# TheCacophonyProject/audio-analysis

Measured on AMD Instinct MI355X. Metric: audio-seconds classified/sec/GPU on 60 s mono; max|delta logit| vs CPU ref, higher is better.
Workload: dtype bf16x3; 1 GPU; config2: 64 windows/step (39 of clip A + 25 of clip B, 60 s 48 kHz mono), htk log-mel n_fft 4096 hop 640 160 mel + model1 CNN; model=model1, global_batch=64, seq_len=144000, parallelism=dp1, pipeline=2 batches in flight on 2 streams, clip_pairs=4 resident clip pairs in rotation, one per step

## Files before the change

audio-analysis_amd/csrc/aa_frontend.hip:

```cpp
#include "aa_common.h"
#include "aa_wavefft.h"

#include <algorithm>
#include <cmath>
#include <cstring>
#include <vector>

namespace aa {

constexpr int kStatSplit = 16;
constexpr int kFpb = 6;

struct FePlan {
    aa_fe_config cfg;
    int T = 0;
    int kmin = 0;
    int kmax = 0;
    int nfblk = 0;
    int nnz = 0;
    float* d_win = nullptr;
    float2* d_tw = nullptr;
    float2* d_tw2 = nullptr;
    int4* d_rows = nullptr;
    float* d_vals = nullptr;
    char* d_cimg = nullptr;
    int cimg_bytes = 0;
    StageTimer timer;
};

enum { FE_STAGE_STATS = 0, FE_STAGE_STFT = 1, FE_STAGE_DB = 2, FE_N_STAGES = 3 };

__global__ __launch_bounds__(256) void fe_stats(const float* __restrict__ pcm,
                                                const aa_window* __restrict__ wins,
                                                int win_len, float4* __restrict__ stats) {
    const int w = blockIdx.y;
    const aa_window d = wins[w];
    const int chunk = (win_len + kStatSplit - 1) / kStatSplit;
    const int i0 = blockIdx.x * chunk;
    const int i1 = min(win_len, i0 + chunk);
    float mn = INFINITY, mx = -INFINITY;
    int bad = 0;
    const int v0 = max(i0, d.pad_left);
    const int v1 = min(i1, d.pad_left + d.n_valid);
    if (i0 < i1 && !(v0 == i0 && v1 >= i1)) { mn = 0.f; mx = 0.f; }
    if (v0 < v1) {
        const float* p = pcm + d.src + (v0 - d.pad_left);
        const int n = v1 - v0;
        const int head = min(n, (int)((16 - ((uintptr_t)p & 15)) & 15) / 4);
        for (int i = threadIdx.x; i < head; i += blockDim.x) {
            float x = p[i];
            bad |= !isfinite(x);
            mn = fminf(mn, x);
            mx = fmaxf(mx, x);
        }
        const int nb = (n - head) / 4;
        const float4* q = reinterpret_cast<const float4*>(p + head);
        constexpr int U = 4;
        for (int i = threadIdx.x; i < nb; i += U * blockDim.x) {
            float4 x[U];
#pragma unroll
            for (int u = 0; u < U; ++u) x[u] = q[min(i + u * (int)blockDim.x, nb - 1)];
#pragma unroll
            for (int u = 0; u < U; ++u) {
                bad |= !isfinite(x[u].x) | !isfinite(x[u].y) | !isfinite(x[u].z) | !isfinite(x[u].w);
                mn = fminf(fminf(mn, x[u].x), fminf(x[u].y, fminf(x[u].z, x[u].w)));
                mx = fmaxf(fmaxf(mx, x[u].x), fmaxf(x[u].y, fmaxf(x[u].z, x[u].w)));
            }
        }
        for (int i = head + nb * 4 + threadIdx.x; i < n; i += blockDim.x) {
            float x = p[i];
            bad |= !isfinite(x);
            mn = fminf(mn, x);
            mx = fmaxf(mx, x);
        }
    }
    __shared__ float smn[4], smx[4];
    __shared__ int sbad[4];
    mn = wave_min(mn);
    mx = wave_max(mx);
    bad = wave_or(bad);
    const int wv = threadIdx.x >> 6;
    if ((threadIdx.x & 63) == 0) { smn[wv] = mn; smx[wv] = mx; sbad[wv] = bad; }
    __syncthreads();
    if (threadIdx.x == 0) {
        for (int k = 1; k < (int)(blockDim.x >> 6); ++k) {
            mn = fminf(mn, smn[k]);
            mx = fmaxf(mx, smx[k]);
            bad |= sbad[k];
        }
        stats[w * kStatSplit + blockIdx.x] = make_float4(mn, mx, (float)bad, 0.f);
    }
}

__device__ __forceinline__ int pidx(int i) { return i + (i >> 3); }

template <int NC, int R, int NT, int NS>
struct Pass {
    static constexpr int NB = NC / R;
    static constexpr int PER = (NB + NT - 1) / NT;
    float2 t[PER][R - 1];
    __device__ __forceinline__ void load(const float2* __restrict__ tw) {
#pragma unroll
        for (int b = 0; b < PER; ++b) {
            const int j = threadIdx.x + b * NT;
            const int k = j % NS;
#pragma unroll
            for (int r = 1; r < R; ++r)
                t[b][r - 1] = tw[(r * k * (NC / (NS * R))) & (NC - 1)];
        }
    }
    __device__ __forceinline__ void run(const float2* __restrict__ src, float2* __restrict__ dst) const {
#pragma unroll
        for (int b = 0; b < PER; ++b) {
            const int j = threadIdx.x + b * NT;
            if (NB % NT == 0 || j < NB) {
                float2 v[R];
#pragma unroll
                for (int r = 0; r < R; ++r) v[r] = src[pidx(j + r * NB)];
                if constexpr (NS > 1) {
#pragma unroll
                    for (int r = 1; r < R; ++r) v[r] = cmul(v[r], t[b][r - 1]);
                }
                if constexpr (R == 8) dft8(v);
                if constexpr (R == 4) dft4(v[0], v[1], v[2], v[3]);
                if constexpr (R == 2) dft2(v[0], v[1]);
                const int k = j % NS;
                const int o = (j / NS) * NS * R + k;
#pragma unroll
                for (int r = 0; r < R; ++r) dst[pidx(o + r * NS)] = v[r];
            }
        }
    }
};

__device__ __forceinline__ float normalize_sample(float x, float lo, float scale, float inv) {
    const float a = __fsub_rn(x, lo);
    const float q0 = __fmul_rn(a, inv);
    const float r = fmaf(-q0, scale, a);
    float y = fmaf(r, inv, q0);
    y = __fadd_rn(y, 0.000001f);
    y = __fsub_rn(y, 0.5f);
    return __fmul_rn(y, 2.0f);
}

enum { PM_GENERAL = 0, PM_ABS = 1, PM_SQUARE = 2 };
template <int PM>
__device__ __forceinline__ float pow_mag(float re, float im, float power) {
    const float m2 = fmaf(re, re, im * im);
    if constexpr (PM == PM_SQUARE) return m2;
    const float mag = __builtin_amdgcn_sqrtf(m2);
    if constexpr (PM == PM_ABS) return mag;
    else return powf(mag, power);
}

template <int NFFT, int PM>
__global__ __launch_bounds__(NFFT / 16) void fe_stft_mel(
    const float* __restrict__ pcm, const aa_window* __restrict__ wins, const float4* __restrict__ stats,
    const float* __restrict__ hann, const float2* __restrict__ tw, const float2* __restrict__ tw2,
    const int4* __restrict__ rows, const float* __restrict__ vals, int nnz, int win_len, int hop, int T,
    int n_mels, int kmin, int kmax, int normalize, float power, int nfblk, int n_items,
    float* __restrict__ melS, float* __restrict__ blkmax) {
    constexpr int NC = NFFT / 2;
    constexpr int NT = NC / 8;
    constexpr int R4 = NC / 512;
    static_assert(NC >= 1024 && NC <= 4096, "NFFT 2048..8192");
    constexpr int KREG = 4;
    extern __shared__ float lds[];
    float* seg = lds;
    const int seg_cap = ((kFpb - 1) * hop + NFFT + 3) & ~3;
    float2* bufA = reinterpret_cast<float2*>(lds + seg_cap);
    constexpr int NCP = NC + NC / 8;
    float2* bufB = bufA + NCP;
    float* melT = reinterpret_cast<float*>(bufB + NCP);
    int4* srows = reinterpret_cast<int4*>(melT + ((n_mels * kFpb + 3) & ~3));
    float* svals = reinterpret_cast<float*>(srows + n_mels);

    const int tid = threadIdx.x;
    float hw[8][2];
#pragma unroll
    for (int r = 0; r < 8; ++r) {
        const int n = tid + r * (NC / 8);
        const float2 h = reinterpret_cast<const float2*>(hann)[n];
        hw[r][0] = h.x;
        hw[r][1] = h.y;
    }
    Pass<NC, 8, NT, 8> p2;
    Pass<NC, 8, NT, 64> p3;
    Pass<NC, R4, NT, 512> p4;
    p2.load(tw);
    p3.load(tw);
    p4.load(tw);
    float2 w2r[KREG];
#pragma unroll
    for (int i = 0; i < KREG; ++i) {
        w2r[i] = tw2[min(kmin + tid + i * NT, kmax)];
    }
    for (int i = tid; i < n_mels; i += NT) srows[i] = rows[i];
    for (int i = tid; i < nnz; i += NT) svals[i] = vals[i];

    __syncthreads();
    for (int item = blockIdx.x; item < n_items; item += gridDim.x) {
    const int w = item / nfblk;
    const int fb = item - w * nfblk;
    const int f0 = fb * kFpb;
    const int nf = min(kFpb, T - f0);
    const int seg_len = (nf - 1) * hop + NFFT;
    const aa_window d = wins[w];
    float lo = INFINITY, hi = -INFINITY;
#pragma unroll
    for (int s = 0; s < kStatSplit; ++s) {
        float4 st = stats[w * kStatSplit + s];
        lo = fminf(lo, st.x);
        hi = fmaxf(hi, st.y);
    }
    const float scale = __fsub_rn(hi, lo);
    const float inv = __fdiv_rn(1.f, scale);

    const int base = f0 * hop - NFFT / 2;
    constexpr int SEGU = 8;
    const long long safe = d.n_valid > 0 ? d.src : 0;
    for (int q0 = 0; q0 < seg_len; q0 += SEGU * NT) {
        float raw[SEGU];
        bool ok[SEGU];
#pragma unroll
        for (int u = 0; u < SEGU; ++u) {
            const int q = q0 + u * NT + tid;
            const int i = base + q;
            const int rel = i - d.pad_left;
            ok[u] = q < seg_len && i >= 0 && i < win_len && rel >= 0 && rel < d.n_valid;
            raw[u] = pcm[ok[u] ? d.src + rel : safe];
        }
#pragma unroll
        for (int u = 0; u < SEGU; ++u) {
            const int q = q0 + u * NT + tid;
            const int i = base + q;
            if (q < seg_len) {
                float v = 0.f;
                if (i >= 0 && i < win_len) {
                    v = ok[u] ? raw[u] : 0.f;
                    if (normalize) v = normalize_sample(v, lo, scale, inv);
                }
                seg[q] = v;
            }
        }
    }
    __syncthreads();

    float bmax = 0.f;
    for (int f = 0; f < nf; ++f) {
        {
            const float* x = seg + f * hop;
            float2 v[8];
#pragma unroll
            for (int r = 0; r < 8; ++r) {
                const int n = tid + r * NT;
                v[r] = make_float2(x[2 * n] * hw[r][0], x[2 * n + 1] * hw[r][1]);
            }
            dft8(v);
#pragma unroll
            for (int r = 0; r < 8; ++r) bufA[pidx(tid * 8 + r)] = v[r];
        }
        __syncthreads();
        p2.run(bufA, bufB);
        __syncthreads();
        p3.run(bufB, bufA);
        __syncthreads();
        p4.run(bufA, bufB);
        __syncthreads();
        const float2* Z = bufB;
        float* Pf = reinterpret_cast<float*>(bufA);
        for (int i = 0; kmin + tid + i * NT <= kmax; ++i) {
            const int k = kmin + tid + i * NT;
            float re, im;
            if (k == 0 || k == NC) {
                const float2 z0 = Z[0];
                re = (k == 0) ? z0.x + z0.y : z0.x - z0.y;
                im = 0.f;
            } else {
                const float2 a = Z[pidx(k)];
                const float2 b = Z[pidx(NC - k)];
                const float2 E = make_float2(0.5f * (a.x + b.x), 0.5f * (a.y - b.y));
                const float2 O = make_float2(0.5f * (a.y + b.y), -0.5f * (a.x - b.x));
                float2 wk;
                if (i < KREG) {
                    wk = w2r[0];
#pragma unroll
                    for (int q = 1; q < KREG; ++q) if (i == q) wk = w2r[q];
                } else {
                    wk = tw2[k];
                }
                const float2 X = cadd(E, cmul(wk, O));
                re = X.x;
                im = X.y;
            }
            Pf[k - kmin] = pow_mag<PM>(re, im, power);
        }
        __syncthreads();
        for (int m = tid; m < n_mels; m += NT) {
            const int4 rw = srows[m];
            const float* wv = svals + rw.z;
            const float* pv = Pf + (rw.x - kmin);
            float s = 0.f;
            for (int i0 = 0; i0 < rw.y; i0 += 16) {
                float a[16], b[16];
#pragma unroll
                for (int i = 0; i < 16; ++i) {
                    const int ii = min(i0 + i, rw.y - 1);
                    a[i] = (i0 + i < rw.y) ? wv[ii] : 0.f;
                    b[i] = pv[ii];
                }
#pragma unroll
                for (int i = 0; i < 16; ++i) s = fmaf(a[i], b[i], s);
            }
            melT[m * kFpb + f] = s;
            bmax = fmaxf(bmax, s);
        }
        __syncthreads();
    }
    const float inv_nm = 1.0f / (float)n_mels;
    for (int idx = tid; idx < nf * n_mels; idx += NT) {
        const int f = (int)(((float)idx + 0.5f) * inv_nm), m = idx - f * n_mels;
        melS[((size_t)w * T + f0 + f) * n_mels + m] = melT[m * kFpb + f];
    }
    __shared__ float red[NT / 64];
    bmax = wave_max(bmax);
    if ((tid & 63) == 0) red[tid >> 6] = bmax;
    __syncthreads();
    if (tid == 0) {
        for (int k = 1; k < NT / 64; ++k) bmax = fmaxf(bmax, red[k]);
        blkmax[w * nfblk + fb] = bmax;
    }
    }
}

__host__ __device__ constexpr int fe_mel_slots(int n_mels) { return (n_mels + 63) / 64 * 64; }

#ifndef AA_FE_WPB
#define AA_FE_WPB 8
#endif
#ifndef AA_FE_MEL_G
#define AA_FE_MEL_G 2
#endif
#ifndef AA_FE_MEL_P
#define AA_FE_MEL_P 1
#endif
constexpr int kWpb = AA_FE_WPB;

constexpr int kFeStampPh = 8;
__device__ unsigned long long* fe_stamps = nullptr;
#define FE_STAMP(k)                                                              \
    if constexpr ((DIAG & 128) != 0) {                                           \
        const unsigned long long tn = __builtin_amdgcn_s_memtime();              \
        st_acc[k] += tn - st_prev;                                               \
        st_prev = tn;                                                            \
    }
template <int PM, int DIAG = 0>
__global__ __launch_bounds__(64 * kWpb) __attribute__((amdgpu_waves_per_eu(kWpb / 2, kWpb / 2))) void fe_stft_mel_4096(
    const float* __restrict__ pcm, const aa_window* __restrict__ wins, const float4* __restrict__ stats,
    const float2* __restrict__ tw, const float2* __restrict__ tw4096, const char* __restrict__ cimg,
    int cimg_bytes, int win_len, int hop, int T, int n_mels, int kmin, int kmax, int normalize, float power,
    int n_frames, float* __restrict__ melF, float* __restrict__ pmax) {
    constexpr int NC = 2048;
    extern __shared__ float lds[];
    const int tid = threadIdx.x;
    const int wave = __builtin_amdgcn_readfirstlane(tid >> 6), lane = tid & 63;
    char* cl = reinterpret_cast<char*>(lds);
    const int4* srows = reinterpret_cast<const int4*>(cl);
    const float* svals = reinterpret_cast<const float*>(srows + fe_mel_slots(n_mels));
    float2* wb = reinterpret_cast<float2*>(cl + cimg_bytes) + wave * kHalf;

    for (int g = wave; g < cimg_bytes / 1024; g += kWpb)
        __builtin_amdgcn_global_load_lds((const __attribute__((address_space(1))) void*)(cimg + g * 1024 + lane * 16),
                                         (__attribute__((address_space(3))) void*)(cl + g * 1024), 16, 0, 0);
    const int k1 = lane >> 1, h = lane & 1;
    float2 t1 = tw[lane];
    float2 t8 = tw[(8 * lane) & (NC - 1)];
    const float2 wk1 = tw4096[k1];
    const float2 te = tw4096[2 * lane], to = tw4096[2 * lane + 1];
    const float2 hwe = make_float2(te.x, -te.y), hwo = make_float2(to.x, -to.y);
    __syncthreads();
    unsigned long long st_acc[kFeStampPh] = {}, st_prev = 0;
    auto load_frame = [&](int fl, float2 (&yy)[32]) {
        const int wl = fl / T;
        const aa_window dl = wins[wl];
        const int i0l = (fl - wl * T) * hop - 2048;
        int l2l = 2 * lane;
        __asm__ volatile("" : "+v"(l2l));
        const __amdgpu_buffer_rsrc_t rs =
            __builtin_amdgcn_make_buffer_rsrc((void*)(pcm + dl.src), 0, dl.n_valid * 4, 0x00020000);
        const int offe = i0l - dl.pad_left + l2l;
        const int v0 = i0l - dl.pad_left;
        if (v0 >= 0 && v0 + 4096 <= dl.n_valid) {
#pragma unroll
            for (int r = 0; r < 32; ++r) {
                const uint2 v = __builtin_bit_cast(uint2, __builtin_amdgcn_raw_buffer_load_b64(rs, (offe + 128 * r) * 4, 0, 0));
                yy[r] = make_float2(__uint_as_float(v.x), __uint_as_float(v.y));
            }
        } else {
            int offo = offe + 1;
            __asm__ volatile("" : "+v"(offo));
#pragma unroll
            for (int r = 0; r < 32; ++r) yy[r] = make_float2(load_view(rs, offe + 128 * r), load_view(rs, offo + 128 * r));
        }
    };

    const int nbx = gridDim.x >> 3;
    const int xcd = blockIdx.x & 7;
    const int f_end = (int)((long long)(xcd + 1) * n_frames / 8);
    const int G = nbx * kWpb;
    const int f_first = (int)((long long)xcd * n_frames / 8) + wave * nbx + (blockIdx.x >> 3);
    for (int fi = f_first; fi < f_end; fi += G) {
        const int w = fi / T;
        const int t = fi - w * T;
        if constexpr ((DIAG & 128) != 0) st_prev = __builtin_amdgcn_s_memtime();
        float apow = 1.f, beta = 0.f;
        if (normalize) {
            float lo = INFINITY, hi = -INFINITY;
#pragma unroll
            for (int s = 0; s < kStatSplit; ++s) {
                const float4 st = stats[w * kStatSplit + s];
                lo = fminf(lo, st.x);
                hi = fmaxf(hi, st.y);
            }
            const float scale = __fsub_rn(hi, lo);
            const float a = __fdiv_rn(2.f, scale);
            apow = PM == PM_SQUARE ? a * a : PM == PM_ABS ? a : powf(a, power);
            beta = fmaf(scale, 0.000001f - 0.5f, -lo);
        }
        const int i0 = t * hop - 2048;
        int l2 = 2 * lane;
        __asm__ volatile("" : "+v"(l2));
        float2 wk = wk1;
        __asm__ volatile("" : "+v"(wk.x), "+v"(wk.y));
        float2 u[32];
        {
            float2 y[32];
            if constexpr ((DIAG & 1) != 0) {
#pragma unroll
                for (int r = 0; r < 32; ++r) y[r] = make_float2((float)(lane + r), (float)(t - r));
            } else {
                load_frame(fi, y);
            }
            if (normalize && (i0 < 0 || i0 + 4096 > win_len)) {
#pragma unroll
                for (int r = 0; r < 32; ++r) {
                    const int i = i0 + l2 + 128 * r;
                    y[r].x = (i >= 0 && i < win_len) ? y[r].x + beta : 0.f;
                    y[r].y = (i + 1 >= 0 && i + 1 < win_len) ? y[r].y + beta : 0.f;
                }
            }
            float2 he = hwe, ho = hwo;
            float hs = lane >= 32 ? -0.5f : 0.5f;
            __asm__ volatile("" : "+v"(he.x), "+v"(he.y), "+v"(ho.x), "+v"(ho.y), "+v"(hs));
#pragma unroll
            for (int r = 0; r < 32; ++r) {
                const float cr = kW32[r][0], sr = -kW32[r][1];
                const float ce = fmaf(he.x, cr, -he.y * sr), co = fmaf(ho.x, cr, -ho.y * sr);
                const float a = (r & 1) ? hs : 0.5f;
                y[r].x *= fmaf(-a, ce, a);
                y[r].y *= fmaf(-a, co, a);
            }
            FE_STAMP(0)
            if constexpr ((DIAG & 4) != 0) {
#pragma unroll
                for (int j = 0; j < 32; ++j) u[j] = y[j];
            } else {
                const unsigned up = lane >= 32 ? 0x80000000u : 0u;
                auto flip = [up](float2 v) {
                    return make_float2(__uint_as_float(__float_as_uint(v.x) ^ up),
                                       __uint_as_float(__float_as_uint(v.y) ^ up));
                };
                dft32(y);
                FE_STAMP(1)
                __asm__ volatile("" : "+v"(t1.x), "+v"(t1.y), "+v"(t8.x), "+v"(t8.y));
                float2 p1[8], p8[4];
                p1[0] = make_float2(1.f, 0.f);
                p1[1] = t1;
#pragma unroll
                for (int i = 2; i < 8; ++i) p1[i] = cmul(p1[i - 1], t1);
                {
                    const float2 q1 = t8, q2 = cmul(t8, t8), q3 = cmul(q2, t8);
                    const bool hi = lane >= 32;
                    p8[0] = hi ? q2 : make_float2(1.f, 0.f);
                    p8[1] = hi ? q3 : q1;
                    p8[2] = hi ? make_float2(1.f, 0.f) : q2;
                    p8[3] = hi ? q1 : q3;
                }
#pragma unroll
                for (int k = 0; k < 32; ++k) {
                    const float2 tk = (k & 7) == 0 ? p8[k >> 3] : cmul(p8[k >> 3], p1[k & 7]);
                    y[dperm(k)] = cmul(y[dperm(k)], tk);
                }
                FE_STAMP(2)
#pragma unroll
                for (int pass = 0; pass < 2; ++pass) {
#pragma unroll
                    for (int k = 0; k < 16; ++k) wb[k * kRow + lane] = y[dperm(16 * pass + k)];
                    wave_sync();
                    const float2* src = wb + (k1 & 15) * kRow + h + 32 * (((k1 >> 4) ^ pass) & 1);
#pragma unroll
                    for (int i = 0; i < 16; ++i) u[16 * pass + i] = src[2 * i];
                    wave_sync();
                }
                FE_STAMP(3)
                dft32(u);
#pragma unroll
                for (int k = 1; k < 32; k += 2) u[dperm(k)] = flip(u[dperm(k)]);
                FE_STAMP(4)
                const float sg = h ? -1.f : 1.f;
#pragma unroll
                for (int j = 0; j < 32; ++j) {
                    const float2 e = u[dperm(j)];
                    const float2 wj = wconst64(j);
                    const float2 g = h ? cmul(wj, e) : e;
                    const float2 rv = make_float2(swap_pair(g.x), swap_pair(g.y));
                    u[dperm(j)] = make_float2(fmaf(sg, g.x, rv.x), fmaf(sg, g.y, rv.y));
                }
                FE_STAMP(5)
            }
        }
        if (h && !(DIAG & 8)) {
#pragma unroll
            for (int j = 0; j < 32; ++j) wb[k1 + 32 * j] = u[dperm(j)];
        }
        wave_sync();
        float* Pt = reinterpret_cast<float*>(wb) + (2 * kHalf - 1);
        if (!(DIAG & 8)) {
            const float2* mb = wb + (32 - k1) - 512 * h;
            float* pk = Pt - k1 - 512 * h - 32 * 15;
            const float r2 = 0.70710678118654752440f;
            const float2 wkh = h ? make_float2(r2 * (wk.x + wk.y), r2 * (wk.y - wk.x)) : wk;
            float pw[16];
            float2 zm[16];
#pragma unroll
            for (int i = 0; i < 8; ++i) zm[i] = mb[32 * (31 - i)];
#pragma unroll
            for (int i = 0; i < 16; ++i) {
                if (i % 8 == 0 && i + 8 < 16) {
#pragma unroll
                    for (int k = i + 8; k < i + 16; ++k) zm[k] = mb[32 * (31 - k)];
                }
                const float2 hiv = u[dperm(16 + i)];
                const float2 oth = make_float2(swap_pair(hiv.x), swap_pair(hiv.y));
                const float2 a = h ? oth : u[dperm(i)];
                const float2 zb = zm[i];
                const float2 b = (i == 0 && k1 == 0 && !h) ? a : zb;
                const float2 E = make_float2(0.5f * (a.x + b.x), 0.5f * (a.y - b.y));
                const float2 O = make_float2(0.5f * (a.y + b.y), -0.5f * (a.x - b.x));
                float2 wj = cmul(wkh, wconst128(i));
                __asm__ volatile("" : "+v"(wj.x), "+v"(wj.y));
                const float2 X = cadd(E, cmul(wj, O));
                pw[i] = pow_mag<PM>(X.x, X.y, power);
            }
            if (!(DIAG & 16)) {
#pragma unroll
                for (int i = 0; i < 16; ++i) pk[32 * (15 - i)] = pw[i];
            }
        }
        wave_sync();
        FE_STAMP(6)
        float fmx = 0.f;
        float* orow = melF + (size_t)fi * n_mels;
        const int nslot = fe_mel_slots(n_mels);
#if AA_FE_MEL_G > 0
        int si0 = lane;
        __asm__ volatile("" : "+v"(si0));
#else
        const int si0 = lane;
#endif
#if AA_FE_MEL_G > 0
        constexpr int G = AA_FE_MEL_G, NP = AA_FE_MEL_P;
        for (int si = si0; si < ((DIAG & 32) ? 0 : nslot); si += 64 * NP) {
            int4 rw[NP];
            const float4* wv[NP];
            const float* pv[NP];
            float4 wa[NP][G];
            float pa[NP][G][4];
#pragma unroll
            for (int q = 0; q < NP; ++q) {
                const int sq = si + 64 * q;
                rw[q] = sq < nslot ? srows[sq] : make_int4(kmin + 3, 0, 0, -1);
                wv[q] = reinterpret_cast<const float4*>(svals + rw[q].z);
                pv[q] = Pt - rw[q].x - (rw[q].y - 1);
                const int glast = max((rw[q].y >> 2) - 1, 0);
#pragma unroll
                for (int g = 0; g < G; ++g) {
                    const int gi = min(g, glast);
                    wa[q][g] = wv[q][gi];
#pragma unroll
                    for (int e = 0; e < 4; ++e) pa[q][g][e] = pv[q][4 * gi + e];
                }
            }
#pragma unroll
            for (int q = 0; q < NP; ++q) {
                float s = 0.f;
#pragma unroll
                for (int g = 0; g < G; ++g) {
                    if (4 * g < rw[q].y) {
                        s = fmaf(wa[q][g].x, pa[q][g][0], s);
                        s = fmaf(wa[q][g].y, pa[q][g][1], s);
                        s = fmaf(wa[q][g].z, pa[q][g][2], s);
                        s = fmaf(wa[q][g].w, pa[q][g][3], s);
                    }
                }
                for (int i = 4 * G; i < rw[q].y; i += 4) {
                    const float4 a = wv[q][i >> 2];
                    s = fmaf(a.x, pv[q][i], s);
                    s = fmaf(a.y, pv[q][i + 1], s);
                    s = fmaf(a.z, pv[q][i + 2], s);
                    s = fmaf(a.w, pv[q][i + 3], s);
                }
                s *= apow;
                if (!(DIAG & 64) && rw[q].w >= 0) orow[rw[q].w] = s;
                fmx = fmaxf(fmx, s);
            }
        }
#else
        for (int si = si0; si < ((DIAG & 32) ? 0 : nslot); si += 64) {
            const int4 rw = srows[si];
            const float4* wv = reinterpret_cast<const float4*>(svals + rw.z);
            const float* pv = Pt - rw.x - (rw.y - 1);
            float s = 0.f;
            for (int i = 0; i < rw.y; i += 4) {
                const float4 a = wv[i >> 2];
                s = fmaf(a.x, pv[i], s);
                s = fmaf(a.y, pv[i + 1], s);
                s = fmaf(a.z, pv[i + 2], s);
                s = fmaf(a.w, pv[i + 3], s);
            }
            s *= apow;
            if (!(DIAG & 64) && rw.w >= 0) orow[rw.w] = s;
            fmx = fmaxf(fmx, s);
        }
#endif
        fmx = wave_max(fmx);
        if (lane == 0 && !(DIAG & 64)) pmax[fi] = fmx;
        wave_sync();
        FE_STAMP(7)
    }
    if constexpr ((DIAG & 128) != 0) {
        const size_t gw = (size_t)blockIdx.x * kWpb + wave;
#pragma unroll
        for (int k = 0; k < kFeStampPh; ++k) fe_stamps[(gw * kFeStampPh + k) * 64 + lane] = st_acc[k];
    }
}

__device__ __forceinline__ float db_value(float v, float ref_db, int db_scale, float amin, float top_db) {
    if (db_scale) {
        v = __fsub_rn(__fmul_rn(10.0f, log10f(fmaxf(amin, v))), ref_db);
        v = fmaxf(v, -top_db);
    }
    return v;
}

__device__ __forceinline__ float window_ref_db(const float* __restrict__ pmax, int nparts, float amin, float* red) {
    float mx = 0.f;
    for (int i = threadIdx.x; i < nparts; i += blockDim.x) mx = fmaxf(mx, pmax[i]);
    mx = wave_max(mx);
    if ((threadIdx.x & 63) == 0) red[threadIdx.x >> 6] = mx;
    __syncthreads();
    mx = red[0];
    for (int k = 1; k < (int)(blockDim.x >> 6); ++k) mx = fmaxf(mx, red[k]);
    return __fmul_rn(10.0f, log10f(fmaxf(amin, mx)));
}

template <typename TO>
__global__ __launch_bounds__(256) void fe_db(const float* __restrict__ melF, const float* __restrict__ pmax,
                                             int nparts, const float4* __restrict__ stats,
                                             const float* __restrict__ band_mean, int n_mels, int T, int tile_t,
                                             int db_scale, float amin, float top_db, int channels, int normalize,
                                             TO* __restrict__ out, int* __restrict__ status) {
    extern __shared__ float tile[];
    __shared__ float red[4];
    const int w = blockIdx.y;
    const int t0 = blockIdx.x * tile_t;
    const int nt = min(tile_t, T - t0);
    const int ld = n_mels + 1;
    const float* src = melF + ((size_t)w * T + t0) * n_mels;
    const int total = nt * n_mels;
    const float inv_nm = 1.0f / (float)n_mels;
    const int tsh = __builtin_ctz(tile_t);
#ifndef AA_FE_DB_U
#define AA_FE_DB_U 8
#endif
    constexpr int U = AA_FE_DB_U;
    float v[U];
#pragma unroll
    for (int u = 0; u < U; ++u) v[u] = src[min(u * 256 + (int)threadIdx.x, total - 1)];
    const float ref_db = window_ref_db(pmax + (size_t)w * nparts, nparts, amin, red);
    if (blockIdx.x == 0 && threadIdx.x == 0 && status) {
        float lo = INFINITY, hi = -INFINITY;
        int bad = 0;
        for (int s = 0; s < kStatSplit; ++s) {
            const float4 st = stats[w * kStatSplit + s];
            lo = fminf(lo, st.x);
            hi = fmaxf(hi, st.y);
            bad |= st.z != 0.f;
        }
        if (normalize && !(hi - lo > 0.f)) bad = 1;
        status[w] = bad ? AA_WIN_NONFINITE : AA_WIN_OK;
    }
    for (int i0 = 0; i0 < total; i0 += U * 256) {
        if (i0 > 0) {
#pragma unroll
            for (int u = 0; u < U; ++u) v[u] = src[min(i0 + u * 256 + (int)threadIdx.x, total - 1)];
        }
#pragma unroll
        for (int u = 0; u < U; ++u) {
            const int idx = i0 + u * 256 + threadIdx.x;
            if (idx < total) {
                const int tt = (int)(((float)idx + 0.5f) * inv_nm), m = idx - tt * n_mels;
                tile[tt * ld + m] = db_value(v[u], ref_db, db_scale, amin, top_db);
            }
        }
    }
    __syncthreads();
    for (int idx = threadIdx.x; idx < n_mels * tile_t; idx += 256) {
        const int m = idx >> tsh, tt = idx & (tile_t - 1);
        if (tt < nt) {
            float v = tile[tt * ld + m];
            if (band_mean) v -= band_mean[(size_t)w * n_mels + m];
            TO* o = out + (((size_t)w * n_mels + m) * T + t0 + tt) * channels;
            for (int c = 0; c < channels; ++c) o[c] = (TO)v;
        }
    }
}

__global__ __launch_bounds__(256) void fe_band_mean(const float* __restrict__ melF, const float* __restrict__ pmax,
                                                    int nparts, int n_mels, int T, int db_scale, float amin,
                                                    float top_db, float* __restrict__ band_mean) {
    __shared__ float red[4];
    const int w = blockIdx.x;
    const float ref_db = window_ref_db(pmax + (size_t)w * nparts, nparts, amin, red);
    const float* src = melF + (size_t)w * T * n_mels;
    for (int m = threadIdx.x; m < n_mels; m += 256) {
        float s = 0.f;
        for (int t = 0; t < T; ++t) s += db_value(src[(size_t)t * n_mels + m], ref_db, db_scale, amin, top_db);
        band_mean[(size_t)w * n_mels + m] = s / (float)T;
    }
}

static size_t fe_lds_bytes(const FePlan& p) {
    const int nc = p.cfg.n_fft / 2;
    const int seg_cap = ((kFpb - 1) * p.cfg.hop + p.cfg.n_fft + 3) & ~3;
    return sizeof(float) * ((size_t)seg_cap + 4 * (size_t)(nc + nc / 8) + (size_t)((p.cfg.n_mels * kFpb + 3) & ~3) + 4 * (size_t)p.cfg.n_mels +
                            (size_t)std::max(p.nnz, 1));
}

template <int NFFT, int PM>
static int launch_stft(const FePlan& p, const float* pcm, const aa_window* wins, int n_win,
                       const float4* stats, float* melS, float* blkmax, hipStream_t st) {
    const size_t lds = fe_lds_bytes(p);
    AA_CHECK(lds <= 150 * 1024, AA_ERR_UNSUPPORTED, "fe: hop %d needs %zu B of LDS", p.cfg.hop, lds);
    AA_DYN_LDS((fe_stft_mel<NFFT, PM>), lds);
    const int n_items = p.nfblk * n_win;
    const int per_cu = std::max(1, (int)((160 * 1024) / (lds + 256)));
    const int grid = std::min(n_items, 256 * per_cu);
    hipLaunchKernelGGL((fe_stft_mel<NFFT, PM>), dim3(grid), dim3(NFFT / 16), lds, st, pcm, wins, stats, p.d_win,
                       p.d_tw, p.d_tw2, p.d_rows, p.d_vals, p.nnz, p.cfg.win_len, p.cfg.hop, p.T,
                       p.cfg.n_mels, p.kmin, p.kmax, p.cfg.normalize, p.cfg.power, p.nfblk, n_items,
                       melS, blkmax);
    AA_LAUNCH_CHECK();
    return AA_OK;
}

static bool fe_fast4096(const FePlan& p) {
    return p.cfg.n_fft == 4096 && p.kmin >= 2 && p.kmax <= 1022 && p.kmin + 64 * (kHalf / 64 - 1) < kHalf &&
           p.kmax - p.kmin + 1 + 3 <= (kHalf / 64 - 1) * 64;
}

static size_t fe_lds_bytes4096(const FePlan& p) {
    return (size_t)p.cimg_bytes + sizeof(float2) * (size_t)kWpb * kHalf;
}

template <int PM>
static int launch_stft4096(const FePlan& p, const float* pcm, const aa_window* wins, int n_win,
                           const float4* stats, float* melS, float* pmax, hipStream_t st) {
    const size_t lds = fe_lds_bytes4096(p);
    AA_CHECK(lds <= 160 * 1024, AA_ERR_UNSUPPORTED, "fe4096: %zu B of LDS", lds);
    AA_DYN_LDS(fe_stft_mel_4096<PM>, lds);
    const int n_frames = p.T * n_win;
    const int per_cu = std::max(1, std::min(2, (int)((160 * 1024) / lds)));
    int grid = std::min((n_frames + kWpb - 1) / kWpb, 256 * per_cu);
    grid = (grid + 7) & ~7;
    hipLaunchKernelGGL(fe_stft_mel_4096<PM>, dim3(grid), dim3(64 * kWpb), lds, st, pcm, wins, stats, p.d_tw,
                       p.d_tw2, p.d_cimg, p.cimg_bytes, p.cfg.win_len, p.cfg.hop, p.T, p.cfg.n_mels, p.kmin,
                       p.kmax, p.cfg.normalize, p.cfg.power, n_frames, melS, pmax);
    AA_LAUNCH_CHECK();
    return AA_OK;
}

struct FeWs {
    float4* stats;
    float* melS;
    float* blkmax;
    float* band_mean;
    size_t bytes;
};

static FeWs fe_ws_layout(const FePlan& p, int n_win, char* base) {
    FeWs w{};
    size_t off = 0;
    w.stats = reinterpret_cast<float4*>(base + off);
    off = align_up(off + sizeof(float4) * (size_t)n_win * kStatSplit, 256);
    w.melS = reinterpret_cast<float*>(base + off);
    off = align_up(off + sizeof(float) * (size_t)n_win * p.cfg.n_mels * p.T, 256);
    w.blkmax = reinterpret_cast<float*>(base + off);
    off = align_up(off + sizeof(float) * (size_t)n_win * p.nfblk, 256);
    w.band_mean = reinterpret_cast<float*>(base + off);
    if (p.cfg.mean_sub) off = align_up(off + sizeof(float) * (size_t)n_win * p.cfg.n_mels, 256);
    w.bytes = off;
    return w;
}

}

using namespace aa;

extern "C" int aa_fe_create(const aa_fe_config* cfg, const float* melfb, void** plan) {
    AA_CHECK(cfg && melfb && plan, AA_ERR_INVALID, "aa_fe_create: null argument");
    const int n = cfg->n_fft;
    AA_CHECK(n == 2048 || n == 4096 || n == 8192, AA_ERR_UNSUPPORTED,
             "aa_fe_create: n_fft %d not supported (power of two 2048..8192)", n);
    AA_CHECK(cfg->hop > 0 && cfg->win_len > 0 && cfg->n_mels > 0 && cfg->channels >= 1 &&
                 (cfg->out_f16 == 0 || cfg->out_f16 == 1),
             AA_ERR_INVALID, "aa_fe_create: bad sizes");
    FePlan* p = new FePlan();
    p->cfg = *cfg;
    p->T = 1 + cfg->win_len / cfg->hop;

    const int nbins = n / 2 + 1;
    std::vector<int4> rows(cfg->n_mels);
    std::vector<float> vals;
    int kmin = nbins, kmax = 0;
    for (int m = 0; m < cfg->n_mels; ++m) {
        const float* r = melfb + (size_t)m * nbins;
        int a = -1, b = -1;
        for (int k = 0; k < nbins; ++k)
            if (r[k] != 0.f) { if (a < 0) a = k; b = k; }
        if (a < 0) { a = 0; b = -1; }
        rows[m] = make_int4(a, b - a + 1, (int)vals.size(), 0);
        for (int k = a; k <= b; ++k) vals.push_back(r[k]);
        if (b >= a) { kmin = std::min(kmin, a); kmax = std::max(kmax, b); }
    }
    if (kmax < kmin) { kmin = 0; kmax = 0; }
    for (auto& r : rows) if (r.y == 0) r.x = kmin;
    p->kmin = kmin;
    p->kmax = kmax;
    p->nnz = (int)vals.size();
    p->nfblk = fe_fast4096(*p) ? p->T : (p->T + kFpb - 1) / kFpb;
    if (vals.empty()) vals.push_back(0.f);
    const int nc = n / 2;
    std::vector<float> win(n);
    for (int i = 0; i < n; ++i) win[i] = (float)(0.5 - 0.5 * std::cos(2.0 * M_PI * i / n));
    std::vector<float2> tw(nc), tw2(nc + 1);
    for (int m = 0; m < nc; ++m) {
        const double a = -2.0 * M_PI * m / nc;
        tw[m] = make_float2((float)std::cos(a), (float)std::sin(a));
    }
    for (int k = 0; k <= nc; ++k) {
        const double a = -2.0 * M_PI * k / n;
        tw2[k] = make_float2((float)std::cos(a), (float)std::sin(a));
    }
    auto up = [](void** d, const void* h, size_t b) -> hipError_t {
        hipError_t e = hipMalloc(d, b);
        if (e != hipSuccess) return e;
        return hipMemcpy(*d, h, b, hipMemcpyHostToDevice);
    };
    hipError_t e = hipSuccess;
    if (e == hipSuccess) e = up((void**)&p->d_win, win.data(), sizeof(float) * n);
    if (e == hipSuccess) e = up((void**)&p->d_tw, tw.data(), sizeof(float2) * nc);
    if (e == hipSuccess) e = up((void**)&p->d_tw2, tw2.data(), sizeof(float2) * (nc + 1));
    if (e == hipSuccess) e = up((void**)&p->d_rows, rows.data(), sizeof(int4) * rows.size());
    if (e == hipSuccess) e = up((void**)&p->d_vals, vals.data(), sizeof(float) * vals.size());
    if (e == hipSuccess && n == 4096) {
        const int nslot = fe_mel_slots(cfg->n_mels);
        std::vector<int4> prow(nslot, make_int4(kmin + 3, 0, 0, -1));
        std::vector<float> pval;
        std::vector<int> order(rows.size());
        for (size_t m = 0; m < rows.size(); ++m) order[m] = (int)m;
        std::stable_sort(order.begin(), order.end(), [&](int a, int b) { return rows[a].y > rows[b].y; });
        std::vector<int> load(64, 0), used(64, 0);
        for (int m : order) {
            int best = -1;
            for (int l = 0; l < 64; ++l)
                if (used[l] < nslot / 64 && (best < 0 || load[l] < load[best])) best = l;
            const int len = (rows[m].y + 3) & ~3, pad = len - rows[m].y;
            prow[best + 64 * used[best]] = make_int4(rows[m].x, len, (int)pval.size(), m);
            load[best] += len;
            ++used[best];
            for (int i = 0; i < len; ++i) pval.push_back(i < pad ? 0.f : vals[rows[m].z + rows[m].y - 1 - (i - pad)]);
        }
        const size_t raw = sizeof(int4) * prow.size() + sizeof(float) * pval.size();
        std::vector<char> img((raw + 1023) / 1024 * 1024, 0);
        memcpy(img.data(), prow.data(), sizeof(int4) * prow.size());
        memcpy(img.data() + sizeof(int4) * prow.size(), pval.data(), sizeof(float) * pval.size());
        p->cimg_bytes = (int)img.size();
        e = up((void**)&p->d_cimg, img.data(), img.size());
    }
    if (e != hipSuccess) {
        set_error("aa_fe_create: %s", hipGetErrorString(e));
        aa_fe_destroy(p);
        return AA_ERR_HIP;
    }
    AA_CHECK(fe_lds_bytes(*p) <= 150 * 1024, AA_ERR_UNSUPPORTED,
             "aa_fe_create: hop %d too large for the LDS segment", cfg->hop);
    *plan = p;
    return AA_OK;
}

extern "C" int aa_fe_destroy(void* plan) {
    FePlan* p = static_cast<FePlan*>(plan);
    if (!p) return AA_OK;
    (void)hipFree(p->d_win);
    (void)hipFree(p->d_tw);
    (void)hipFree(p->d_tw2);
    (void)hipFree(p->d_rows);
    (void)hipFree(p->d_vals);
    (void)hipFree(p->d_cimg);
    p->timer.release();
    delete p;
    return AA_OK;
}

extern "C" int aa_fe_n_frames(const void* plan) {
    return plan ? static_cast<const FePlan*>(plan)->T : -1;
}

extern "C" size_t aa_fe_workspace_bytes(const void* plan, int32_t max_windows) {
    if (!plan || max_windows < 0) return 0;
    return fe_ws_layout(*static_cast<const FePlan*>(plan), max_windows, nullptr).bytes;
}

extern "C" int aa_fe_run(void* plan, const float* pcm, int64_t pcm_len, const aa_window* windows,
                         int32_t n_win, void* out, int32_t* win_status, void* workspace,
                         size_t workspace_bytes, void* stream) {
    FePlan* p = static_cast<FePlan*>(plan);
    AA_CHECK(p && pcm && windows && out, AA_ERR_INVALID, "aa_fe_run: null argument");
    AA_CHECK(n_win >= 0, AA_ERR_INVALID, "aa_fe_run: n_win < 0");
    (void)pcm_len;
    if (n_win == 0) return AA_OK;
    constexpr int32_t CHUNK = 32768;
    if (n_win > CHUNK) {
        const size_t ob = (size_t)p->cfg.n_mels * p->T * p->cfg.channels * (p->cfg.out_f16 ? 2 : 4);
        for (int32_t c0 = 0; c0 < n_win; c0 += CHUNK) {
            const int32_t nc = std::min(CHUNK, n_win - c0);
            const int rc = aa_fe_run(plan, pcm, pcm_len, windows + c0, nc, static_cast<char*>(out) + c0 * ob,
                                     win_status ? win_status + c0 : nullptr, workspace, workspace_bytes, stream);
            if (rc != AA_OK) return rc;
        }
        return AA_OK;
    }
    FeWs ws = fe_ws_layout(*p, n_win, static_cast<char*>(workspace));
    AA_CHECK(workspace && workspace_bytes >= ws.bytes, AA_ERR_WORKSPACE,
             "aa_fe_run: workspace %zu < %zu bytes", workspace_bytes, ws.bytes);
    hipStream_t st = static_cast<hipStream_t>(stream);
    hipEvent_t e0;
    int rc = p->timer.begin(FE_STAGE_STATS, st, &e0);
    if (rc != AA_OK) return rc;
    hipLaunchKernelGGL(fe_stats, dim3(kStatSplit, n_win), dim3(256), 0, st, pcm, windows,
                       p->cfg.win_len, ws.stats);
    AA_LAUNCH_CHECK();
    if ((rc = p->timer.end(FE_STAGE_STATS, st, e0)) != AA_OK) return rc;
    if ((rc = p->timer.begin(FE_STAGE_STFT, st, &e0)) != AA_OK) return rc;
    const int pm = p->cfg.power == 2.f ? PM_SQUARE : p->cfg.power == 1.f ? PM_ABS : PM_GENERAL;
#define AA_FE_PM(PM)                                                                                    \
    if (fe_fast4096(*p)) {                                                                              \
        rc = launch_stft4096<PM>(*p, pcm, windows, n_win, ws.stats, ws.melS, ws.blkmax, st);            \
    } else switch (p->cfg.n_fft) {                                                                      \
        case 2048: rc = launch_stft<2048, PM>(*p, pcm, windows, n_win, ws.stats, ws.melS, ws.blkmax, st); break; \
        case 4096: rc = launch_stft<4096, PM>(*p, pcm, windows, n_win, ws.stats, ws.melS, ws.blkmax, st); break; \
        default: rc = launch_stft<8192, PM>(*p, pcm, windows, n_win, ws.stats, ws.melS, ws.blkmax, st); break;   \
    }
    if (pm == PM_SQUARE) { AA_FE_PM(PM_SQUARE) }
    else if (pm == PM_ABS) { AA_FE_PM(PM_ABS) }
    else { AA_FE_PM(PM_GENERAL) }
#undef AA_FE_PM
    if (rc != AA_OK) return rc;
    if ((rc = p->timer.end(FE_STAGE_STFT, st, e0)) != AA_OK) return rc;
    if ((rc = p->timer.begin(FE_STAGE_DB, st, &e0)) != AA_OK) return rc;
    if (p->cfg.mean_sub) {
        hipLaunchKernelGGL(fe_band_mean, dim3(n_win), dim3(256), 0, st, ws.melS, ws.blkmax, p->nfblk,
                           p->cfg.n_mels, p->T, p->cfg.db_scale, p->cfg.amin, p->cfg.top_db, ws.band_mean);
        AA_LAUNCH_CHECK();
    }
#ifndef AA_FE_DB_TILE
#define AA_FE_DB_TILE 8
#endif
    static_assert((AA_FE_DB_TILE & (AA_FE_DB_TILE - 1)) == 0, "fe_db indexes its tile by shifts");
    int tile_t = AA_FE_DB_TILE;
    while (tile_t > 1 && (size_t)tile_t * (p->cfg.n_mels + 1) * 4 > 65536) tile_t >>= 1;
    if (p->cfg.out_f16) {
        hipLaunchKernelGGL(fe_db<_Float16>, dim3((p->T + tile_t - 1) / tile_t, n_win), dim3(256),
                           (size_t)tile_t * (p->cfg.n_mels + 1) * 4, st, ws.melS, ws.blkmax, p->nfblk, ws.stats,
                           p->cfg.mean_sub ? ws.band_mean : nullptr, p->cfg.n_mels, p->T, tile_t, p->cfg.db_scale,
                           p->cfg.amin, p->cfg.top_db, p->cfg.channels, p->cfg.normalize, (_Float16*)out, win_status);
    } else {
        hipLaunchKernelGGL(fe_db<float>, dim3((p->T + tile_t - 1) / tile_t, n_win), dim3(256),
                           (size_t)tile_t * (p->cfg.n_mels + 1) * 4, st, ws.melS, ws.blkmax, p->nfblk, ws.stats,
                           p->cfg.mean_sub ? ws.band_mean : nullptr, p->cfg.n_mels, p->T, tile_t, p->cfg.db_scale,
                           p->cfg.amin, p->cfg.top_db, p->cfg.channels, p->cfg.normalize, (float*)out, win_status);
    }
    AA_LAUNCH_CHECK();
    return p->timer.end(FE_STAGE_DB, st, e0);
}

extern "C" int aa_fe_n_stages(const void* plan) { return plan ? FE_N_STAGES : -1; }

extern "C" int aa_fe_stage_info(const void* plan, int32_t stage, char* name, int32_t name_len,
                                double* flops_per_item, double* bytes_per_item) {
    const FePlan* p = static_cast<const FePlan*>(plan);
    AA_CHECK(p && stage >= 0 && stage < FE_N_STAGES, AA_ERR_INVALID, "aa_fe_stage_info: bad stage");
    const double N = p->cfg.n_fft, L = p->cfg.win_len, T = p->T, M = p->cfg.n_mels;
    double fl = 0, by = 0;
    const char* nm = "";
    switch (stage) {
        case FE_STAGE_STATS: nm = "fe_stats"; fl = 2 * L; by = 4 * L; break;
        case FE_STAGE_STFT:
            nm = fe_fast4096(*p) ? "fe_stft_mel_4096" : "fe_stft_mel";
            fl = T * (2.5 * N * std::log2(N) + N + 3 * (N / 2 + 1) + 2.0 * p->nnz) + 5 * L;
            by = 4 * L + 4 * M * T;
            break;
        default: nm = "fe_db"; fl = 3 * M * T; by = M * T * (4 + (p->cfg.out_f16 ? 2 : 4) * p->cfg.channels); break;
    }
    if (name && name_len > 0) snprintf(name, name_len, "%s", nm);
    if (flops_per_item) *flops_per_item = fl;
    if (bytes_per_item) *bytes_per_item = by;
    return AA_OK;
}

extern "C" int aa_fe_set_timing(void* plan, uint32_t stage_mask) {
    FePlan* p = static_cast<FePlan*>(plan);
    AA_CHECK(p, AA_ERR_INVALID, "aa_fe_set_timing: null plan");
    p->timer.mask = stage_mask;
    return AA_OK;
}

extern "C" int aa_fe_stage_time(void* plan, int32_t stage, double* total_ms, int64_t* count) {
    FePlan* p = static_cast<FePlan*>(plan);
    AA_CHECK(p && stage >= 0 && stage < FE_N_STAGES, AA_ERR_INVALID, "aa_fe_stage_time: bad stage");
    return p->timer.collect(stage, total_ms, count);
}
```

Measured before the change: 276,600 audio-s/s.

## Use cross-lane permutes for real-FFT split and retile dB transpose kernel

In the 4096-point STFT kernel, the real-FFT split step no longer goes through a wave-local LDS buffer with a barrier. Mirrored bins are now exchanged with ds_bpermute, and the 0.5 scaling is folded into the normalization power constant. The Hann window loop is halved by applying both symmetric halves in one pass. The dB/transpose kernel is retiled to 16 mel bands by 256 time frames with a static LDS tile, so output writes run along time contiguously and the float division used for index recovery is gone. The risks are more permute traffic, register pressure, and subtle numerical changes from the changed scaling order.

```diff
diff --git a/audio-analysis_amd/csrc/aa_frontend.hip b/audio-analysis_amd/csrc/aa_frontend.hip
--- a/audio-analysis_amd/csrc/aa_frontend.hip
+++ b/audio-analysis_amd/csrc/aa_frontend.hip
@@ -151,6 +151,16 @@
     const float mag = __builtin_amdgcn_sqrtf(m2);
     if constexpr (PM == PM_ABS) return mag;
     else return powf(mag, power);
+}
+
+template <int PM>
+__device__ __forceinline__ float split_pow(float2 a, float2 b, float2 w, float power) {
+#pragma clang fp contract(off)
+    constexpr float c = PM == PM_GENERAL ? 0.5f : 1.f;
+    const float sx = a.x + b.x, dy = a.y - b.y;
+    const float ox = c * (a.y + b.y), oy = -c * (a.x - b.x);
+    const float tre = fmaf(ox, w.x, -(oy * w.y)), tim = fmaf(oy, w.x, ox * w.y);
+    return pow_mag<PM>(fmaf(c, sx, tre), fmaf(c, dy, tim), power);
 }
 
 template <int NFFT, int PM>
@@ -361,6 +371,7 @@
     int cimg_bytes, int win_len, int hop, int T, int n_mels, int kmin, int kmax, int normalize, float power,
     int n_frames, float* __restrict__ melF, float* __restrict__ pmax) {
     constexpr int NC = 2048;
+    constexpr float kPowFold = PM == PM_SQUARE ? 0.25f : PM == PM_ABS ? 0.5f : 1.f;
     extern __shared__ float lds[];
     const int tid = threadIdx.x;
     const int wave = __builtin_amdgcn_readfirstlane(tid >> 6), lane = tid & 63;
@@ -375,7 +386,9 @@
     const int k1 = lane >> 1, h = lane & 1;
     float2 t1 = tw[lane];
     float2 t8 = tw[(8 * lane) & (NC - 1)];
-    const float2 wk1 = tw4096[k1];
+    const int kq = h ? (32 - k1) & 31 : k1;
+    const int pull = 4 * (2 * ((32 - k1) & 31) + (h ^ 1));
+    const float2 wk1 = tw4096[kq];
     const float2 te = tw4096[2 * lane], to = tw4096[2 * lane + 1];
     const float2 hwe = make_float2(te.x, -te.y), hwo = make_float2(to.x, -to.y);
     __syncthreads();
@@ -413,7 +426,7 @@
         const int w = fi / T;
         const int t = fi - w * T;
         if constexpr ((DIAG & 128) != 0) st_prev = __builtin_amdgcn_s_memtime();
-        float apow = 1.f, beta = 0.f;
+        float apow = kPowFold, beta = 0.f;
         if (normalize) {
             float lo = INFINITY, hi = -INFINITY;
 #pragma unroll
@@ -424,7 +437,7 @@
             }
             const float scale = __fsub_rn(hi, lo);
             const float a = __fdiv_rn(2.f, scale);
-            apow = PM == PM_SQUARE ? a * a : PM == PM_ABS ? a : powf(a, power);
+            apow = PM == PM_SQUARE ? (a * a) * kPowFold : PM == PM_ABS ? a * kPowFold : powf(a, power);
             beta = fmaf(scale, 0.000001f - 0.5f, -lo);
         }
         const int i0 = t * hop - 2048;
@@ -453,12 +466,14 @@
             float hs = lane >= 32 ? -0.5f : 0.5f;
             __asm__ volatile("" : "+v"(he.x), "+v"(he.y), "+v"(ho.x), "+v"(ho.y), "+v"(hs));
 #pragma unroll
-            for (int r = 0; r < 32; ++r) {
+            for (int r = 0; r < 16; ++r) {
                 const float cr = kW32[r][0], sr = -kW32[r][1];
                 const float ce = fmaf(he.x, cr, -he.y * sr), co = fmaf(ho.x, cr, -ho.y * sr);
                 const float a = (r & 1) ? hs : 0.5f;
                 y[r].x *= fmaf(-a, ce, a);
                 y[r].y *= fmaf(-a, co, a);
+                y[r + 16].x *= fmaf(a, ce, a);
+                y[r + 16].y *= fmaf(a, co, a);
             }
             FE_STAMP(0)
             if constexpr ((DIAG & 4) != 0) {
@@ -519,42 +534,39 @@
                 FE_STAMP(5)
             }
         }
-        if (h && !(DIAG & 8)) {
-#pragma unroll
-            for (int j = 0; j < 32; ++j) wb[k1 + 32 * j] = u[dperm(j)];
-        }
-        wave_sync();
         float* Pt = reinterpret_cast<float*>(wb) + (2 * kHalf - 1);
         if (!(DIAG & 8)) {
-            const float2* mb = wb + (32 - k1) - 512 * h;
-            float* pk = Pt - k1 - 512 * h - 32 * 15;
+            float* pk = Pt - kq - 512 * h - 32 * 15;
             const float r2 = 0.70710678118654752440f;
             const float2 wkh = h ? make_float2(r2 * (wk.x + wk.y), r2 * (wk.y - wk.x)) : wk;
-            float pw[16];
-            float2 zm[16];
-#pragma unroll
-            for (int i = 0; i < 8; ++i) zm[i] = mb[32 * (31 - i)];
+            const float cj = h ? -1.f : 1.f;
+            float2 prev = u[dperm(0)];
+#pragma unroll
+            for (int j = 0; j < 16; ++j)
+                if (lane == 1) u[dperm(j)] = u[dperm(j + 1)];
+            constexpr int PB = 8;
+            float2 gt[PB];
 #pragma unroll
             for (int i = 0; i < 16; ++i) {
-                if (i % 8 == 0 && i + 8 < 16) {
-#pragma unroll
-                    for (int k = i + 8; k < i + 16; ++k) zm[k] = mb[32 * (31 - k)];
-                }
-                const float2 hiv = u[dperm(16 + i)];
-                const float2 oth = make_float2(swap_pair(hiv.x), swap_pair(hiv.y));
-                const float2 a = h ? oth : u[dperm(i)];
-                const float2 zb = zm[i];
-                const float2 b = (i == 0 && k1 == 0 && !h) ? a : zb;
-                const float2 E = make_float2(0.5f * (a.x + b.x), 0.5f * (a.y - b.y));
-                const float2 O = make_float2(0.5f * (a.y + b.y), -0.5f * (a.x - b.x));
+                if (i % PB == 0) {
+                    __builtin_amdgcn_sched_barrier(0);
+#pragma unroll
+                    for (int k = 0; k < PB; ++k) {
+                        const float2 snd = h ? u[dperm(31 - i - k)] : u[dperm(16 + i + k)];
+                        gt[k] = make_float2(
+                            __int_as_float(__builtin_amdgcn_ds_bpermute(pull, __float_as_int(snd.x))),
+                            __int_as_float(__builtin_amdgcn_ds_bpermute(pull, __float_as_int(snd.y))));
+                    }
+                }
+                const float2 got = gt[i % PB];
+                const float2 a = h ? u[dperm(15 - i)] : u[dperm(i)];
+                const float2 b = lane == 0 ? prev : got;
+                prev = got;
                 float2 wj = cmul(wkh, wconst128(i));
+                wj.y *= cj;
                 __asm__ volatile("" : "+v"(wj.x), "+v"(wj.y));
-                const float2 X = cadd(E, cmul(wj, O));
-                pw[i] = pow_mag<PM>(X.x, X.y, power);
-            }
-            if (!(DIAG & 16)) {
-#pragma unroll
-                for (int i = 0; i < 16; ++i) pk[32 * (15 - i)] = pw[i];
+                const float pw = split_pow<PM>(a, b, wj, power);
+                if (!(DIAG & 16)) pk[32 * (15 - i)] = pw;
             }
         }
         wave_sync();
@@ -664,29 +676,28 @@
     return __fmul_rn(10.0f, log10f(fmaxf(amin, mx)));
 }
 
+constexpr int kDbBg = 16;
+constexpr int kDbTc = 256;
+constexpr int kDbLd = kDbTc + 4;
 template <typename TO>
 __global__ __launch_bounds__(256) void fe_db(const float* __restrict__ melF, const float* __restrict__ pmax,
                                              int nparts, const float4* __restrict__ stats,
-                                             const float* __restrict__ band_mean, int n_mels, int T, int tile_t,
+                                             const float* __restrict__ band_mean, int n_mels, int T, int n_bg,
                                              int db_scale, float amin, float top_db, int channels, int normalize,
                                              TO* __restrict__ out, int* __restrict__ status) {
-    extern __shared__ float tile[];
+    __shared__ float tile[kDbBg * kDbLd];
     __shared__ float red[4];
     const int w = blockIdx.y;
-    const int t0 = blockIdx.x * tile_t;
-    const int nt = min(tile_t, T - t0);
-    const int ld = n_mels + 1;
-    const float* src = melF + ((size_t)w * T + t0) * n_mels;
-    const int total = nt * n_mels;
-    const float inv_nm = 1.0f / (float)n_mels;
-    const int tsh = __builtin_ctz(tile_t);
-#ifndef AA_FE_DB_U
-#define AA_FE_DB_U 8
-#endif
-    constexpr int U = AA_FE_DB_U;
+    const int tc = blockIdx.x / n_bg, bg = blockIdx.x - tc * n_bg;
+    const int t0 = tc * kDbTc, nt = min(kDbTc, T - t0);
+    const int m0 = bg * kDbBg, nb = min(kDbBg, n_mels - m0);
+    constexpr int FP = 256 / kDbBg;
+    constexpr int U = kDbTc / FP;
+    const int b = threadIdx.x & (kDbBg - 1), f = threadIdx.x / kDbBg;
+    const float* src = melF + ((size_t)w * T + t0) * n_mels + m0 + min(b, nb - 1);
     float v[U];
 #pragma unroll
-    for (int u = 0; u < U; ++u) v[u] = src[min(u * 256 + (int)threadIdx.x, total - 1)];
+    for (int u = 0; u < U; ++u) v[u] = src[(size_t)min(u * FP + f, nt - 1) * n_mels];
     const float ref_db = window_ref_db(pmax + (size_t)w * nparts, nparts, amin, red);
     if (blockIdx.x == 0 && threadIdx.x == 0 && status) {
         float lo = INFINITY, hi = -INFINITY;
@@ -700,28 +711,17 @@
         if (normalize && !(hi - lo > 0.f)) bad = 1;
         status[w] = bad ? AA_WIN_NONFINITE : AA_WIN_OK;
     }
-    for (int i0 = 0; i0 < total; i0 += U * 256) {
-        if (i0 > 0) {
-#pragma unroll
-            for (int u = 0; u < U; ++u) v[u] = src[min(i0 + u * 256 + (int)threadIdx.x, total - 1)];
-        }
-#pragma unroll
-        for (int u = 0; u < U; ++u) {
-            const int idx = i0 + u * 256 + threadIdx.x;
-            if (idx < total) {
-                const int tt = (int)(((float)idx + 0.5f) * inv_nm), m = idx - tt * n_mels;
-                tile[tt * ld + m] = db_value(v[u], ref_db, db_scale, amin, top_db);
-            }
-        }
-    }
+#pragma unroll
+    for (int u = 0; u < U; ++u)
+        if (u * FP + f < nt) tile[b * kDbLd + u * FP + f] = db_value(v[u], ref_db, db_scale, amin, top_db);
     __syncthreads();
-    for (int idx = threadIdx.x; idx < n_mels * tile_t; idx += 256) {
-        const int m = idx >> tsh, tt = idx & (tile_t - 1);
-        if (tt < nt) {
-            float v = tile[tt * ld + m];
-            if (band_mean) v -= band_mean[(size_t)w * n_mels + m];
-            TO* o = out + (((size_t)w * n_mels + m) * T + t0 + tt) * channels;
-            for (int c = 0; c < channels; ++c) o[c] = (TO)v;
+    for (int r = 0; r < nb; ++r) {
+        const float mean = band_mean ? band_mean[(size_t)w * n_mels + m0 + r] : 0.f;
+        TO* o = out + (((size_t)w * n_mels + m0 + r) * T + t0) * channels;
+        for (int t = threadIdx.x; t < nt; t += 256) {
+            float x = tile[r * kDbLd + t];
+            if (band_mean) x -= mean;
+            for (int c = 0; c < channels; ++c) o[(size_t)t * channels + c] = (TO)x;
         }
     }
 }
@@ -984,22 +984,17 @@
                            p->cfg.n_mels, p->T, p->cfg.db_scale, p->cfg.amin, p->cfg.top_db, ws.band_mean);
         AA_LAUNCH_CHECK();
     }
-#ifndef AA_FE_DB_TILE
-#define AA_FE_DB_TILE 8
-#endif
-    static_assert((AA_FE_DB_TILE & (AA_FE_DB_TILE - 1)) == 0, "fe_db indexes its tile by shifts");
-    int tile_t = AA_FE_DB_TILE;
-    while (tile_t > 1 && (size_t)tile_t * (p->cfg.n_mels + 1) * 4 > 65536) tile_t >>= 1;
+    const int n_bg = (p->cfg.n_mels + kDbBg - 1) / kDbBg, n_tc = (p->T + kDbTc - 1) / kDbTc;
     if (p->cfg.out_f16) {
-        hipLaunchKernelGGL(fe_db<_Float16>, dim3((p->T + tile_t - 1) / tile_t, n_win), dim3(256),
-                           (size_t)tile_t * (p->cfg.n_mels + 1) * 4, st, ws.melS, ws.blkmax, p->nfblk, ws.stats,
-                           p->cfg.mean_sub ? ws.band_mean : nullptr, p->cfg.n_mels, p->T, tile_t, p->cfg.db_scale,
-                           p->cfg.amin, p->cfg.top_db, p->cfg.channels, p->cfg.normalize, (_Float16*)out, win_status);
+        hipLaunchKernelGGL(fe_db<_Float16>, dim3(n_bg * n_tc, n_win), dim3(256), 0, st, ws.melS, ws.blkmax,
+                           p->nfblk, ws.stats, p->cfg.mean_sub ? ws.band_mean : nullptr, p->cfg.n_mels, p->T, n_bg,
+                           p->cfg.db_scale, p->cfg.amin, p->cfg.top_db, p->cfg.channels, p->cfg.normalize,
+                           (_Float16*)out, win_status);
     } else {
-        hipLaunchKernelGGL(fe_db<float>, dim3((p->T + tile_t - 1) / tile_t, n_win), dim3(256),
-                           (size_t)tile_t * (p->cfg.n_mels + 1) * 4, st, ws.melS, ws.blkmax, p->nfblk, ws.stats,
-                           p->cfg.mean_sub ? ws.band_mean : nullptr, p->cfg.n_mels, p->T, tile_t, p->cfg.db_scale,
-                           p->cfg.amin, p->cfg.top_db, p->cfg.channels, p->cfg.normalize, (float*)out, win_status);
+        hipLaunchKernelGGL(fe_db<float>, dim3(n_bg * n_tc, n_win), dim3(256), 0, st, ws.melS, ws.blkmax,
+                           p->nfblk, ws.stats, p->cfg.mean_sub ? ws.band_mean : nullptr, p->cfg.n_mels, p->T, n_bg,
+                           p->cfg.db_scale, p->cfg.amin, p->cfg.top_db, p->cfg.channels, p->cfg.normalize,
+                           (float*)out, win_status);
     }
     AA_LAUNCH_CHECK();
     return p->timer.end(FE_STAGE_DB, st, e0);
```

Result: no change. 279,300 audio-s/s (median of 6 runs) (+1.0%).
